# thodson-usgs/discontinuum

Hardware: AMD Instinct MI355X
Metric: GP fits/sec (NLL+grad step) at n=8192 d=3, 1/2/4/8 MI355X (higher is better)
Workload: dtype f64

## Files before the change

discontinuum_amd/_lib.py:

```python
from __future__ import annotations

import ctypes as C
import os

_HERE = os.path.dirname(os.path.abspath(__file__))
LIB_PATH = os.path.join(_HERE, "libdgp_hip.so")

F64, F32 = 0, 1
MODEL_LOADEST, MODEL_RATING = 0, 1
OUT_NLL, OUT_QUAD, OUT_LOGDET, OUT_INFO, OUT_DTHETA, OUT_SUM_DR, OUT_DR_W0, OUT_SUM_DNOISE, OUT_LEN = 0, 1, 2, 3, 4, 28, 29, 31, 32
BUF_XT, BUF_A, BUF_T, BUF_S, BUF_Z, BUF_ALPHA = range(6)
BUF_SCAL = 7
OPT_LAUUM64_MAX_TILES, OPT_SYRK_SLOTS, OPT_TRTRI_SMALL, OPT_REFINE, OPT_SYRK_ORDER, OPT_LAUUM_ORDER, OPT_CHAIN_YIELD, OPT_FUSED_GRAD, OPT_GROUP_GEMM = range(9)
TIME_GRAM, TIME_POTRF, TIME_SYRK_SUM, TIME_SYRK_N, TIME_TRTRI, TIME_LAUUM, TIME_SOLVE, TIME_GRAD, TIME_SYRK_FLOP, TIME_COUNT = range(10)


class DGPLibraryError(RuntimeError):
    pass


class DGPError(RuntimeError):
    def __init__(self, code, where, msg):
        super().__init__(f"{where} failed with code {code}: {msg}")
        self.code = code


_vp, _i, _i64, _sz = C.c_void_p, C.c_int, C.c_int64, C.c_size_t
_dp = C.POINTER(C.c_double)

SIGNATURES = {
    "dgp_version": (_i, []),
    "dgp_last_error": (C.c_char_p, []),
    "dgp_model_ntheta": (_i, [_i, _i]),
    "dgp_composite_define": (_i, [C.POINTER(_i), _i, C.POINTER(_i)]),
    "dgp_padded_n": (_i64, [_i64]),
    "dgp_plan_create": (_i, [_i, _i, _i64, _i, C.POINTER(_vp)]),
    "dgp_plan_destroy": (_i, [_vp]),
    "dgp_plan_workspace_bytes": (_sz, [_vp]),
    "dgp_plan_set_workspace": (_i, [_vp, _vp, _sz]),
    "dgp_plan_set_lookahead": (_i, [_vp, _i]),
    "dgp_plan_set_option": (_i, [_vp, _i, _i64]),
    "dgp_plan_get_option": (_i, [_vp, _i, C.POINTER(_i64)]),
    "dgp_plan_set_batch": (_i, [_vp, _i]),
    "dgp_plan_batch": (_i, [_vp]),
    "dgp_plan_set_site_sizes": (_i, [_vp, C.POINTER(C.c_int64), _vp]),
    "dgp_plan_set_dr_weights": (_i, [_vp, _vp]),
    "dgp_dist_last_error": (C.c_char_p, []),
    "dgp_dist_create": (_i, [_i, _i, _i64, _i, _i, _i, _i, C.POINTER(_vp)]),
    "dgp_dist_destroy": (_i, [_vp]),
    "dgp_dist_padded_n": (_i64, [_vp]),
    "dgp_dist_groups": (_i, [_vp]),
    "dgp_dist_slab_columns": (_i64, [_vp]),
    "dgp_dist_workspace_bytes": (_sz, [_vp]),
    "dgp_dist_panel_elems": (_sz, [_vp, _i]),
    "dgp_dist_set_workspace": (_i, [_vp, _vp, _sz]),
    "dgp_dist_set_inputs": (_i, [_vp, _vp, _vp]),
    "dgp_dist_gram": (_i, [_vp, _dp, _vp, _vp]),
    "dgp_dist_factor": (_i, [_vp, _i, _vp, _vp]),
    "dgp_dist_update": (_i, [_vp, _i, _vp, _i, _i, _vp]),
    "dgp_dist_invert": (_i, [_vp, _i, _vp, _vp]),
    "dgp_dist_status": (_i, [_vp, _vp, _vp]),
    "dgp_dist_solve_partial": (_i, [_vp, _vp, _vp, _vp]),
    "dgp_dist_alpha_partial": (_i, [_vp, _vp, _vp, _vp]),
    "dgp_dist_residual": (_i, [_vp, _dp, _vp, _vp, _vp, _vp, _vp, _vp]),
    "dgp_dist_pack_inverse": (_i, [_vp, _i, _vp, _vp]),
    "dgp_dist_product": (_i, [_vp, _i, _vp, _vp]),
# ... 63 lines not shown
```

discontinuum_amd/csrc/dgp_api.hip:

```cpp
#include <mutex>
#include <new>
#include <stdio.h>
#include <stdlib.h>
#include <string.h>
#include <utility>
#include <vector>

#include "../../include/dgp_hip.h"
#include "dgp_common.h"
#include "dgp_internal.h"

using namespace dgp;

static thread_local char g_err[256] = "";
static int fail(int code, const char* msg) {
  snprintf(g_err, sizeof(g_err), "%s", msg);
  return code;
}
static int hipfail(hipError_t e, const char* where) {
  snprintf(g_err, sizeof(g_err), "%s: %s", where, hipGetErrorString(e));
  return (int)e;
}

struct PinnedRing {
// ... 228 lines not shown
  p->z = p->ws + L.z;
  p->alpha = p->ws + L.alpha;
  p->gpart = p->ws + L.gpart;
  p->spart = p->ws + L.spart;
  p->scal = p->ws + L.scal;
  p->info = (int*)(p->ws + L.info);
  p->snap = p->ws + L.snap;
  p->pre = pre_scratch_bytes(p->B) ? (void*)(p->ws + L.total * (size_t)p->B) : nullptr;
  p->pre2 = p->pre ? (void*)((char*)p->pre + align_up(pre_scratch_bytes(p->B))) : nullptr;
  p->nsite = nullptr;
  p->dr_w = nullptr;
  if (p->B > 1) {
    p->nsite = (int*)(p->ws + L.total * (size_t)p->B + 2 * align_up(pre_scratch_bytes(p->B)));
    delete[] p->nsite_host;
    p->nsite_host = new (std::nothrow) int[(size_t)p->B];
    if (!p->nsite_host) return fail(DGP_E_ARG, "dgp_plan_set_workspace: out of host memory");
    for (int b = 0; b < p->B; ++b) p->nsite_host[b] = (int)p->n;
    hipError_t e = hipMemcpy(p->nsite, p->nsite_host, sizeof(int) * (size_t)p->B, hipMemcpyHostToDevice);
    if (e != hipSuccess) return hipfail(e, "dgp_plan_set_workspace: hipMemcpy");
  }
  p->have_inputs = p->have_factor = 0;
  return 0;
}

int dgp_plan_set_option(dgp_plan* p, int key, int64_t value) {
  if (!p) return fail(DGP_E_ARG, "dgp_plan_set_option: null plan");
  switch (key) {
    case DGP_OPT_LAUUM64_MAX_TILES:
      if (value < 0 || value > (1 << 30)) return fail(DGP_E_ARG, "dgp_plan_set_option: value out of range");
      p->tune.lauum64_max_tiles = (int)value;
      return 0;
    case DGP_OPT_SYRK_SLOTS:
      if (value < 1 || value > (1 << 20)) return fail(DGP_E_ARG, "dgp_plan_set_option: value out of range");
      p->tune.syrk_slots = (int)value;
      return 0;
    case DGP_OPT_TRTRI_SMALL:
      if (value < 0) return fail(DGP_E_ARG, "dgp_plan_set_option: value out of range");
      p->tune.trtri_small = (long)value;
      return 0;
    case DGP_OPT_SYRK_ORDER:
    case DGP_OPT_LAUUM_ORDER:
      if (value < 0 || value > 64) return fail(DGP_E_ARG, "dgp_plan_set_option: value out of range");
      (key == DGP_OPT_SYRK_ORDER ? p->tune.syrk_super : p->tune.lauum_super) = (int)value;
      return 0;
    case DGP_OPT_CHAIN_YIELD:
      p->tune.chain_yield = value ? 1 : 0;
      return 0;
    case DGP_OPT_FUSED_GRAD:
      p->tune.fused_grad = value ? 1 : 0;
      return 0;
    case DGP_OPT_GROUP_GEMM:
      p->tune.group_gemm = value ? 1 : 0;
      return 0;
    case DGP_OPT_REFINE:
      if (p->dtype != DGP_F32 && value) return fail(DGP_E_ARG, "dgp_plan_set_option: refinement applies to float32 plans");
      p->refine = value ? 1 : 0;
      return 0;
    default:
      return fail(DGP_E_ARG, "dgp_plan_set_option: unknown option");
  }
}
int dgp_plan_get_option(const dgp_plan* p, int key, int64_t* value) {
  if (!p || !value) return fail(DGP_E_ARG, "dgp_plan_get_option: null argument");
  switch (key) {
    case DGP_OPT_LAUUM64_MAX_TILES: *value = p->tune.lauum64_max_tiles; return 0;
    case DGP_OPT_SYRK_SLOTS: *value = p->tune.syrk_slots; return 0;
    case DGP_OPT_TRTRI_SMALL: *value = p->tune.trtri_small; return 0;
    case DGP_OPT_REFINE: *value = p->refine; return 0;
    case DGP_OPT_SYRK_ORDER: *value = p->tune.syrk_super; return 0;
    case DGP_OPT_LAUUM_ORDER: *value = p->tune.lauum_super; return 0;
    case DGP_OPT_CHAIN_YIELD: *value = p->tune.chain_yield; return 0;
    case DGP_OPT_FUSED_GRAD: *value = p->tune.fused_grad; return 0;
    case DGP_OPT_GROUP_GEMM: *value = p->tune.group_gemm; return 0;
    default: return fail(DGP_E_ARG, "dgp_plan_get_option: unknown option");
  }
}

int dgp_plan_set_lookahead(dgp_plan* p, int level) {
  if (!p) return fail(DGP_E_ARG, "null plan");
  p->lookahead = level ? default_lookahead() : 0;
  p->early = level >= 2 && !getenv("DGP_NO_EARLY_TRTRI");
  return 0;
}

size_t dgp_plan_site_stride_bytes(const dgp_plan* p) { return p ? layout(p).total : 0; }

int dgp_plan_buffer(const dgp_plan* p, int which, void** dev_ptr, int64_t* ld) {
  if (!p || !dev_ptr || !p->ws) return fail(DGP_E_ARG, "dgp_plan_buffer: null / no workspace");
  void* q = nullptr;
  switch (which) {
    case DGP_BUF_XT: q = p->Xt; break;
    case DGP_BUF_A: q = p->A; break;
    case DGP_BUF_T: q = p->Tm; break;
    case DGP_BUF_S: q = p->S; break;
    case DGP_BUF_Z: q = p->z; break;
    case DGP_BUF_ALPHA: q = p->alpha; break;
    case DGP_BUF_INFO: q = p->info; break;
    case DGP_BUF_SCAL: q = p->scal; break;
    default: return fail(DGP_E_ARG, "dgp_plan_buffer: unknown buffer");
  }
  *dev_ptr = q;
  if (ld) *ld = p->N;
  return 0;
}

}

struct StreamSet {
  hipStream_t bulk = nullptr, rest = nullptr, early = nullptr;
};
static StreamSet* stream_set(hipStream_t caller) {
  static std::mutex mtx;
  static std::vector<std::pair<std::pair<int, hipStream_t>, StreamSet*>> sets;
  int dev = 0;
  if (hipGetDevice(&dev) != hipSuccess) return nullptr;
  std::lock_guard<std::mutex> lock(mtx);
  for (auto& e : sets)
    if (e.first.first == dev && e.first.second == caller) return e.second;
  StreamSet* st = new (std::nothrow) StreamSet();
  if (!st) return nullptr;
  sets.push_back({{dev, caller}, st});
  return st;
}
static int make_stream(hipStream_t* out, bool high) {
  if (*out) return 0;
  int least = 0, greatest = 0;
// ... 844 lines not shown
```

discontinuum_amd/csrc/dgp_chol.hip:

```cpp
#include <stdlib.h>
#include <string.h>
#include <mutex>
#include "dgp_diag.h"
#include "dgp_gemm.h"
#include "dgp_gemm_dma.h"
#include "dgp_internal.h"

namespace dgp {

static constexpr int NB = DGP_TILE;
static constexpr int SMID_TABLE = 4096;
template <typename T>
struct Prefetch {
  static constexpr bool F64 = sizeof(T) == 8;
  static constexpr int LAUUM = F64 ? 2 : 4, TRTRI = F64 ? 1 : 4, SYRK = F64 ? 1 : 2;
};

#define DGP_INFO_CHAIN_TIMEOUT (-7)
#define CHAIN_WAIT_TICKS 200000000LL
__device__ __forceinline__ bool chain_reached(const int* word, int value) {
  return __hip_atomic_load(word, __ATOMIC_RELAXED, __HIP_MEMORY_SCOPE_AGENT) >= value;
}
__device__ __forceinline__ bool chain_wait(const int* w0, int v0, const int* w1, int v1, int* info) {
  __shared__ int chain_ok;
  if (threadIdx.x == 0) {
    int ok = 1;
    if (!(chain_reached(w0, v0) && (w1 == nullptr || chain_reached(w1, v1)))) {
      const long long t0 = wall_clock64();
      while (!(chain_reached(w0, v0) && (w1 == nullptr || chain_reached(w1, v1)))) {
        if (__hip_atomic_load(info + CHAIN_ABORT, __ATOMIC_RELAXED, __HIP_MEMORY_SCOPE_AGENT) != 0) {
          ok = 0;
          break;
        }
        if (wall_clock64() - t0 > CHAIN_WAIT_TICKS) {
          atomicCAS(info, 0, DGP_INFO_CHAIN_TIMEOUT);
          __hip_atomic_store(info + CHAIN_ABORT, 1, __ATOMIC_RELAXED, __HIP_MEMORY_SCOPE_AGENT);
          ok = 0;
          break;
        }
        __builtin_amdgcn_s_sleep(8);
      }
    }
    chain_ok = ok;
  }
  __syncthreads();
  __builtin_amdgcn_fence(__ATOMIC_ACQUIRE, "agent");
  return chain_ok != 0;
}

template <typename T>
__global__ __launch_bounds__(256, 2) void trsm_kernel(T* __restrict__ A, const T* __restrict__ Tinv, long ld, int k,
                                                      long bs, int* __restrict__ wait_info = nullptr, int wait_value = 0) {
  if (wait_info && !chain_wait(wait_info + CHAIN_DIAG_DONE, wait_value, nullptr, 0, wait_info)) return;
  A = site(A, bs);
  Tinv = site(Tinv, bs);
  using G = TileGemm<T, true, true, 64, 128>;
  __shared__ T smem[G::SMEM_ELEMS];
  __builtin_amdgcn_s_setprio(3);
  const long row0 = (long)(k + 1) * NB + (long)blockIdx.x * 64;
// ... 31 lines not shown
  typename G::acc_t keep[G::MI][G::NI];
  constexpr bool STREAM = (CMODE & 1) != 0, WIDE = (CMODE & 2) != 0;
  trailing_begin<T, G, K::DMA, STREAM, WIDE>(acc, keep, C, ld);
  if constexpr (POLITE)
    K::run_hooked(A + row0 * ld + (long)k * NB, ld, A + col0 * ld + (long)k * NB, ld, nk * (NB / 16), smem, acc, YieldHook{yield_word, me, yield_copy});
  else
    K::run(A + row0 * ld + (long)k * NB, ld, A + col0 * ld + (long)k * NB, ld, nk * (NB / 16), smem, acc);
  trailing_end<T, G, K::DMA, STREAM, WIDE>(acc, keep, C, ld);
}

template <typename T, bool POLITE = false, int CMODE = 0, int RING = 3>
__global__ __launch_bounds__(256, (TileCore<T, true, true>::OCC)) void syrk_kernel(T* __restrict__ A, long ld, int k, int nk, int jbeg, int nfull,
                                                                                   int split, long bs, int nt = 0, int super = 0,
                                                                                   const unsigned* yield_word = nullptr) {
  A = site(A, bs);
  __shared__ T smem[TileCore<T, true, true, 128, 128, 1, true, false, RING>::SMEM_ELEMS];
  static_assert(TileCore<T, true, true, 64, 128>::SMEM_ELEMS <= TileCore<T, true, true, 128, 128, 1, true, false, RING>::SMEM_ELEMS &&
                    TileCore<T, true, true, 64, 64>::SMEM_ELEMS <= TileCore<T, true, true, 128, 128, 1, true, false, RING>::SMEM_ELEMS,
                "the cut remainder's register-staged tiles must fit the ring's LDS");
  __shared__ unsigned yield_copy[POLITE ? 4 * 64 : 1];
  const int b = (int)blockIdx.x;
  int bi, bj;
  if (b < nfull) {
    if (super > 0) super_decode(xcd_remap(b, nfull), nt, super, bi, bj);
    else tri_decode(xcd_remap(b, nfull), bi, bj);
    syrk_tile<T, 128, 128, POLITE, CMODE, RING>(A, ld, k, nk, (long)(bi + jbeg) * NB, (long)(bj + jbeg) * NB, smem, yield_word, POLITE ? cu_code() : 0u,
                                   yield_copy + (POLITE ? 64 * __builtin_amdgcn_readfirstlane((int)threadIdx.x >> 6) : 0));
    return;
  }
  const int sub = b - nfull;
  if (super > 0) super_decode(nfull + sub / split, nt, super, bi, bj);
  else tri_decode(nfull + sub / split, bi, bj);
  const long row0 = (long)(bi + jbeg) * NB, col0 = (long)(bj + jbeg) * NB;
  const int part = sub % split;
  if (split == 2) {
    syrk_tile<T, 64, 128, false, CMODE>(A, ld, k, nk, row0 + 64 * part, col0, smem);
  } else {
    if (bi == bj && part == 1) return;
    syrk_tile<T, 64, 64, false, CMODE>(A, ld, k, nk, row0 + 64 * (part >> 1), col0 + 64 * (part & 1), smem);
  }
}

const Tuning& default_tuning() {
  static const Tuning t = [] {
    Tuning v;
    v.lauum64_max_tiles = getenv("DGP_LAUUM64") ? atoi(getenv("DGP_LAUUM64")) : 1000;
    v.syrk_slots = getenv("DGP_SYRK_SLOTS") ? atoi(getenv("DGP_SYRK_SLOTS")) : 512;
    v.trtri_small = getenv("DGP_TRTRI_SMALL") ? atol(getenv("DGP_TRTRI_SMALL")) : 1024;
    v.syrk_super = getenv("DGP_SYRK_ORDER") ? atoi(getenv("DGP_SYRK_ORDER")) : 0;
    v.lauum_super = getenv("DGP_LAUUM_ORDER") ? atoi(getenv("DGP_LAUUM_ORDER")) : 0;
    v.chain_yield = getenv("DGP_CHAIN_YIELD") ? atoi(getenv("DGP_CHAIN_YIELD")) : 1;
    v.fused_grad = getenv("DGP_FUSED_GRAD") ? atoi(getenv("DGP_FUSED_GRAD")) : 0;
    v.group_gemm = getenv("DGP_GROUP_GEMM") ? atoi(getenv("DGP_GROUP_GEMM")) : 0;
    if (v.syrk_slots < 1) v.syrk_slots = 1;
    return v;
  }();
  return t;
}
struct SyrkShape {
  int nfull, split;
  unsigned grid;
  explicit SyrkShape(int ntiles, int slots = 512) {
    if (slots < 1) slots = 1;
    const double cost[5] = {0, 1.0, 0.55, 0, 0.30};
    const int whole = ntiles / slots * slots, rem = ntiles - whole;
    nfull = ntiles;
    split = 1;
    double best = (ntiles + slots - 1) / slots * cost[1];
    for (int g = 2; g <= 4; g += 2) {
      const double c = whole / slots * cost[1] + (g * rem + slots - 1) / slots * cost[g];
      if (rem > 0 && c < best - 1e-9) {
        best = c;
        nfull = whole;
        split = g;
      }
    }
    grid = (unsigned)(nfull + split * (ntiles - nfull));
  }
};

template <typename T>
__global__ __launch_bounds__(256, 2) void syrk_col_kernel(T* __restrict__ A, long ld, int k, int nk, int jcol, int nbk,
                                                          int ncol, long bs) {
  using G = TileGemm<T, true, true, 64, 64>;
  __shared__ T smem[G::SMEM_ELEMS];
  __builtin_amdgcn_s_setprio(3);
  A += (long)((int)blockIdx.z / ncol) * bs;
  const int jc = jcol + (int)blockIdx.z % ncol;
  if ((int)blockIdx.x >= 2 * (nbk - jc)) return;
  const long row0 = (long)jc * NB + (long)blockIdx.x * 64;
  const long col0 = (long)jc * NB + (long)blockIdx.y * 64;
  if (col0 > row0 + 63) return;
  typename G::acc_t acc[G::MI][G::NI];
  T* C = A + row0 * ld + col0;
  typename G::acc_t keep[G::MI][G::NI];
  trailing_begin<T, G>(acc, keep, C, ld);
  G::run(A + row0 * ld + (long)k * NB, ld, A + col0 * ld + (long)k * NB, ld, nk * (NB / 16), smem, acc);
  trailing_end<T, G>(acc, keep, C, ld);
}

template <typename T, int CMODE = 0>
__global__ __launch_bounds__(256, (TileCore<T, true, true>::OCC)) void syrk_col128_kernel(T* __restrict__ A, long ld, int k, int nk, int jcol,
                                                                                          int nbk, int ncol, long bs) {
  __shared__ T smem[TileCore<T, true, true>::SMEM_ELEMS];
  A += (long)((int)blockIdx.z / ncol) * bs;
  const int jc = jcol + (int)blockIdx.z % ncol;
  if ((int)blockIdx.x >= nbk - jc) return;
  syrk_tile<T, 128, 128, false, CMODE>(A, ld, k, nk, (long)(jc + (int)blockIdx.x) * NB, (long)jc * NB, smem);
}

struct DeviceOnce {
  std::mutex mtx;
  bool seen[64] = {false};
  template <typename F>
  hipError_t run(F&& configure) {
    int dev = 0;
    if (hipGetDevice(&dev) != hipSuccess || dev < 0 || dev >= 64) return configure();
    std::lock_guard<std::mutex> lock(mtx);
    if (seen[dev]) return hipSuccess;
    const hipError_t e = configure();
    if (e == hipSuccess) seen[dev] = true;
    return e;
  }
};
static bool f32_diag64() {
  static const bool v = [] {
    const char* e = getenv("DGP_F32_DIAG64");
    return e ? atoi(e) != 0 : false;
  }();
  return v;
}
static bool yields(const Batch& bt) { return bt.B == 1 && bt.tuning().chain_yield != 0; }
template <typename T>
static void launch_bulk(T* A, long N, int k, int nk, int jbeg, const SyrkShape& sh, int nt, int* info, hipStream_t s, const Batch& bt) {
  const int nbk = (int)(N / NB);
  const dim3 grid(sh.grid, 1, (unsigned)bt.B);
  static const int pad_env = getenv("DGP_BULK_LDS_PAD") ? std::min(16384, std::max(0, atoi(getenv("DGP_BULK_LDS_PAD")))) : 14336;
  const size_t pad = (bt.B == 1 && nbk >= 40 && nbk <= 160) ? (size_t)pad_env : 0;
  static const int cmode_env = getenv("DGP_BULK_C") ? atoi(getenv("DGP_BULK_C")) & 3 : DGP_BULK_C_DEFAULT;
  const int cmode = sizeof(T) == 8 ? cmode_env : (cmode_env & 1);
  const unsigned* yw = reinterpret_cast<const unsigned*>(info + CHAIN_YIELD);
  static const int ring_env = getenv("DGP_BULK_RING") ? atoi(getenv("DGP_BULK_RING")) : 3;
  static const int pad_batch = getenv("DGP_BULK_PAD_BATCH") ? std::min(65536, std::max(0, atoi(getenv("DGP_BULK_PAD_BATCH")))) : 0;
  if (bt.B >= 4 && bt.tuning().group_gemm && bt.W != nullptr && ring_env == 2) {
    syrk_kernel<T, false, 0, 2><<<grid, 256, (size_t)pad_batch, s>>>(A, N, k, nk, jbeg, sh.nfull, sh.split, bt.ws, nt, bt.tuning().syrk_super, nullptr);
    return;
  }
  const size_t lds_pad = (bt.B >= 4 && pad_batch > 0) ? (size_t)pad_batch : pad;
#define DGP_LAUNCH_BULK(POLITE_, CM_)                                                                                              \
  syrk_kernel<T, POLITE_, CM_><<<grid, 256, lds_pad, s>>>(A, N, k, nk, jbeg, sh.nfull, sh.split, bt.ws, nt, bt.tuning().syrk_super, \
                                                         POLITE_ ? yw : nullptr)
  if (yields(bt)) {
    switch (cmode) {
      case 1: DGP_LAUNCH_BULK(true, 1); break;
      case 2: DGP_LAUNCH_BULK(true, 2); break;
      case 3: DGP_LAUNCH_BULK(true, 3); break;
      default: DGP_LAUNCH_BULK(true, 0);
    }
  } else {
    switch (cmode) {
      case 1: DGP_LAUNCH_BULK(false, 1); break;
      case 2: DGP_LAUNCH_BULK(false, 2); break;
      case 3: DGP_LAUNCH_BULK(false, 3); break;
      default: DGP_LAUNCH_BULK(false, 0);
    }
  }
#undef DGP_LAUNCH_BULK
}
template <typename TS, typename TC>
static void launch_diag_as(TS* A, long N, long k0, TS* Tinv, TS* logdet, int* info, hipStream_t s, Batch bt, bool init,
                           double* logdet_hi, int done_index, int done_value) {
  const size_t bytes = potrf_diag_fast_smem<TC>();
  static DeviceOnce configured;
  (void)configured.run([&] {
    return hipFuncSetAttribute(reinterpret_cast<const void*>(&potrf_diag_fast_kernel<TS, TC>),
                               hipFuncAttributeMaxDynamicSharedMemorySize, (int)bytes);
  });
  potrf_diag_fast_kernel<TS, TC><<<dim3(1, 1, (unsigned)bt.B), 256, bytes, s>>>(
      A, N, k0, Tinv, logdet, info, bt.ws, bt.ws * (long)sizeof(TS) / (long)sizeof(int), init ? 1 : 0, POTRF_INFO_INTS, logdet_hi,
      done_index, done_value, yields(bt) ? CHAIN_YIELD : -1);
}
template <typename T>
static double* logdet_hi_slot(T* logdet) {
  return sizeof(T) == 4 ? reinterpret_cast<double*>(logdet + 2) : nullptr;
}
template <typename T>
static void launch_diag(T* A, long N, long k0, T* Tinv, T* logdet, int* info, hipStream_t s, Batch bt, bool init = false,
                        int done_index = -1, int done_value = 0) {
  if (sizeof(T) == 4 && f32_diag64())
    launch_diag_as<T, double>(A, N, k0, Tinv, logdet, info, s, bt, init, logdet_hi_slot(logdet), done_index, done_value);
  else
    launch_diag_as<T, T>(A, N, k0, Tinv, logdet, info, s, bt, init, logdet_hi_slot(logdet), done_index, done_value);
}

template <typename T>
__global__ __launch_bounds__(256, (TileCore<T, true, true>::OCC)) void trsm_group_kernel(T* __restrict__ A, const T* __restrict__ Tm, long ld,
                                                                                         int k0, int G, long bs) {
  A = site(A, bs);
  Tm = site(Tm, bs);
  using K = TileCore<T, true, true, 128, 128, 1>;
  using Gm = typename K::G;
  __shared__ T smem[K::SMEM_ELEMS];
  T* Arow = A + (long)(k0 + G + (int)blockIdx.x) * NB * ld + (long)k0 * NB;
  const T* TD = Tm + (long)k0 * NB * ld + (long)k0 * NB;
#pragma unroll 1
  for (int j = G - 1; j >= 0; --j) {
    typename Gm::acc_t acc[Gm::MI][Gm::NI];
    Gm::zero(acc);
    K::run(Arow, ld, TD + (long)j * NB * ld, ld, (j + 1) * (NB / 16), smem, acc);
    T* out = Arow + (long)j * NB;
    K::foreach (acc, [&](int r, int c, T& v) { out[(long)r * ld + c] = v; });
  }
}
template <typename T>
static void trtri_group(const T* L, T* Tm, T* W, long N, int k0, int G, hipStream_t s, Batch bt);

template <typename T>
int potrf(T* A, long N, T* Tinv, T* logdet, int* info, int lookahead, hipStream_t s, hipStream_t s2, hipEvent_t* ev,
          hipEvent_t* syrk_ev, int* n_syrk, double* syrk_flop, int nck, const int* ck_blocks, hipEvent_t* ck_ev,
          void (*on_ck)(void*, int), void* ck_ctx, Batch bt, int q_stop, PotrfCarry* carry) {
  const int nbk = (int)(N / NB);
  int ck_next = carry ? carry->ck_next : 0;
  auto checkpoint = [&](int cols_final) {
    while (ck_next < nck && ck_blocks[ck_next] <= cols_final) {
      hipEventRecord(ck_ev[ck_next], s);
      if (on_ck) on_ck(ck_ctx, ck_next);
      ++ck_next;
    }
  };
  int ns = 0;
  double flop = 0.0;
  const unsigned Bz = (unsigned)bt.B;
  auto tri = [](int m) { return (unsigned)(m * (m + 1) / 2); };
  const double tile_flop = 2.0 * NB * NB * NB;
  if (!lookahead || nbk < 4 || s2 == nullptr || ev == nullptr) {
    for (int k = 0; k < nbk; ++k) {
      launch_diag<T>(A, N, (long)k * NB, Tinv, logdet, info, s, bt, k == 0);
      if (k + 1 < nbk) {
        trsm_kernel<T><<<dim3(2 * (nbk - k - 1), 1, Bz), 256, 0, s>>>(A, Tinv, N, k, bt.ws);
        if (syrk_ev) hipEventRecord(syrk_ev[2 * ns], s);
        {
          const SyrkShape sh((int)tri(nbk - k - 1), bt.tuning().syrk_slots / bt.B);
          syrk_kernel<T><<<dim3(sh.grid, 1, Bz), 256, 0, s>>>(A, N, k, 1, k + 1, sh.nfull, sh.split, bt.ws, nbk - k - 1, bt.tuning().syrk_super);
        }
        if (syrk_ev) hipEventRecord(syrk_ev[2 * ns + 1], s);
        flop += tile_flop * tri(nbk - k - 1) * bt.B;
        ++ns;
      }
    }
    checkpoint(nbk);
    if (n_syrk) *n_syrk = ns;
    if (syrk_flop) *syrk_flop = flop;
    return (int)hipGetLastError();
  }
  {
    const int G = lookahead < 2 ? 2 : (lookahead > 8 ? 8 : lookahead);
    hipEvent_t* P = ev;
    hipEvent_t* U = ev + nbk;
    const int Q = (nbk + G - 1) / G;
    const int Qrun = (q_stop >= 0 && q_stop < Q) ? q_stop : Q;
    for (int q = 0; q < Qrun; ++q) {
      const int k0 = G * q, ncol = nbk - k0 < G ? nbk - k0 : G;
      if (q >= 2) hipStreamWaitEvent(s, U[q - 2], 0);
      if (q >= 1) {
        static const int col128 = getenv("DGP_COL128") ? atoi(getenv("DGP_COL128")) : 4;
        if (bt.B >= col128) {
          static const int ccol = getenv("DGP_COL_C") ? atoi(getenv("DGP_COL_C")) & 3 : DGP_COL_C_DEFAULT;
          const dim3 cgrid(nbk - k0, 1, ncol * Bz);
          switch (sizeof(T) == 8 ? ccol : (ccol & 1)) {
            case 1: syrk_col128_kernel<T, 1><<<cgrid, 256, 0, s>>>(A, N, k0 - G, G, k0, nbk, ncol, bt.ws); break;
            case 2: syrk_col128_kernel<T, 2><<<cgrid, 256, 0, s>>>(A, N, k0 - G, G, k0, nbk, ncol, bt.ws); break;
            case 3: syrk_col128_kernel<T, 3><<<cgrid, 256, 0, s>>>(A, N, k0 - G, G, k0, nbk, ncol, bt.ws); break;
            default: syrk_col128_kernel<T, 0><<<cgrid, 256, 0, s>>>(A, N, k0 - G, G, k0, nbk, ncol, bt.ws);
          }
        }
        else syrk_col_kernel<T><<<dim3(2 * (nbk - k0), 2, ncol * Bz), 256, 0, s>>>(A, N, k0 - G, G, k0, nbk, ncol, bt.ws);
      }
      if (q >= 1 && k0 + G < nbk) {
        hipEventRecord(P[q - 1], s);
        hipStreamWaitEvent(s2, P[q - 1], 0);
        if (syrk_ev) hipEventRecord(syrk_ev[2 * ns], s2);
        {
          const SyrkShape sh((int)tri(nbk - k0 - G), bt.tuning().syrk_slots / bt.B);
          launch_bulk<T>(A, N, k0 - G, G, k0 + G, sh, nbk - k0 - G, info, s2, bt);
        }
        if (syrk_ev) hipEventRecord(syrk_ev[2 * ns + 1], s2);
        flop += (double)G * tile_flop * tri(nbk - k0 - G) * bt.B;
        ++ns;
        hipEventRecord(U[q - 1], s2);
      }
      const bool group_gemm = bt.tuning().group_gemm && bt.W != nullptr && ncol == G && k0 + G < nbk && (G & (G - 1)) == 0 && G >= 4 &&
                              nck == 0;
      const int kend = group_gemm ? k0 + G : nbk;
      for (int h = 0; h < ncol; ++h) {
        const int k = k0 + h;
        if (h >= 1) syrk_col_kernel<T><<<dim3(2 * (kend - k), 2, Bz), 256, 0, s>>>(A, N, k0, h, k, kend, 1, bt.ws);
        launch_diag<T>(A, N, (long)k * NB, Tinv, logdet, info, s, bt, k == 0);
        if (k + 1 < kend) trsm_kernel<T><<<dim3(2 * (kend - k - 1), 1, Bz), 256, 0, s>>>(A, Tinv, N, k, bt.ws);
        if (!group_gemm) checkpoint(k + 1);
      }
      if (group_gemm) {
        trtri_group<T>(A, Tinv, (T*)bt.W, N, k0, G, s, bt);
        trsm_group_kernel<T><<<dim3((unsigned)(nbk - k0 - G), 1, Bz), 256, 0, s>>>(A, Tinv, N, k0, G, bt.ws);
        checkpoint(k0 + G);
      }
    }
    if (Qrun == Q) checkpoint(nbk);
// ... 923 lines not shown
```

discontinuum_amd/csrc/dgp_internal.h:

```cpp
#pragma once
#include <hip/hip_runtime.h>
#include <stdint.h>

#define DGP_TILE_HOST 128

namespace dgp {

inline long round_up(long n, long q) { return (n + q - 1) / q * q; }

#define DGP_MAX_BATCH_HOST 8
#define DGP_MAX_BATCH_SITES 1024
struct Tuning {
  int lauum64_max_tiles;
  int syrk_slots;
  long trtri_small;
  int syrk_super;
  int lauum_super;
  int chain_yield;
  int fused_grad;
  int group_gemm;
};
const Tuning& default_tuning();
struct Batch {
  int B = 1;
  long ws = 0;
  const int* ns = nullptr;
  const Tuning* tune = nullptr;
  void* W = nullptr;
  const Tuning& tuning() const { return tune ? *tune : default_tuning(); }
};
int model_ntheta(int model, int d);
int composite_define(const int* spec, int nspec);
bool composite_select(int model, int d);

template <typename T>
int pack_x(const T* X, int n, int d, long N, T* Xt, hipStream_t s, Batch bt = Batch());
template <typename T>
int gram_sym(int model, int d, const T* Xt, long N, int n, const double* theta, const T* noise, T* K, hipStream_t s,
             Batch bt = Batch(), void* pre_scratch = nullptr ,
             void* pre_staging = nullptr ,
             long k_stride = -1 , long noise_stride = -1 ,
             bool pre_ready = false );
template <typename T>
int gram_cross(int model, int d, const T* Xt, long N, int n, const T* Xst, long M, int m, const double* theta,
               T* Ks, hipStream_t s, Batch bt = Batch(), long wbs = 0, void* pre_scratch = nullptr, void* pre_staging = nullptr);
template <typename T>
int gram_diag(int model, int d, const T* Xst, long M, int m, const double* theta, T* kss, hipStream_t s, Batch bt = Batch(),
              long wbs = 0, void* pre_scratch = nullptr);
template <typename T>
int gram_grad(int model, int d, const T* Xt, long N, int n, const double* theta, const T* S, const T* alpha,
              T* partials, T* dtheta, hipStream_t s, Batch bt = Batch(), long dtheta_stride = 0,
              void* pre_scratch = nullptr, bool pre_ready = false ,
              void* pre_staging = nullptr);
size_t pre_scratch_bytes(int B);
template <typename TS>
int gram_residual(int model, int d, const TS* Xt, long N, int n, const double* theta, const TS* noise, const TS* r,
                  const TS* alpha, double* part, double* rho64, TS* rho32, hipStream_t s, Batch bt, long ps, long rs,
                  void* pre_scratch, void* pre_staging);
size_t gram_residual_scratch_bytes(long N);
long gram_grad_partials(long N);
bool lauum_grad_applies(int model, long N, const Batch& bt);
template <typename T>
int lauum_grad(int model, int d, const T* Tm, long N, T* S, const T* Xt, int n, const double* theta, const T* alpha, T* partials,
               T* dtheta, hipStream_t s, Batch bt, long dtheta_stride, void* pre_scratch, bool pre_ready, void* pre_staging);
template <typename T>
int mean_vjp_grad(int model, int d, const T* Xt, long N, int n, const T* Xst, long Mp, int m, const double* theta,
                  const T* alpha, const T* beta, const T* wts, T* partials, T* dtheta, hipStream_t s, Batch bt = Batch(),
                  long wbs = 0, long dstride = 0, void* pre_scratch = nullptr, void* pre_staging = nullptr);
template <typename T>
int gemv_rows(const T* Ks, long N, long Mp, int m, const T* w, T* out, hipStream_t s, int B = 1, long wbs = 0);

struct PotrfCarry {
  int ck_next = 0, ns = 0;
  double flop = 0.0;
};
// ... 87 lines not shown
```

include/dgp_hip.h:

```cpp
#ifndef DGP_HIP_H
#define DGP_HIP_H
#include <stddef.h>
#include <stdint.h>

#ifdef __cplusplus
extern "C" {
#endif

#define DGP_F64 0
#define DGP_F32 1
#define DGP_MODEL_LOADEST 0
#define DGP_MODEL_RATING 1

#define DGP_E_ARG (-1)
#define DGP_E_MODEL (-2)
#define DGP_E_WORKSPACE (-3)
#define DGP_E_STATE (-4)

#define DGP_OUT_NLL 0
#define DGP_OUT_QUAD 1
#define DGP_OUT_LOGDET 2
#define DGP_OUT_INFO 3
#define DGP_OUT_DTHETA 4
#define DGP_OUT_SUM_DR 28
#define DGP_OUT_DR_W0 29
#define DGP_OUT_SUM_DNOISE 31
#define DGP_OUT_LEN 32

#define DGP_BUF_XT 0
#define DGP_BUF_A 1
#define DGP_BUF_T 2
#define DGP_BUF_S 3
#define DGP_BUF_Z 4
#define DGP_BUF_ALPHA 5
#define DGP_BUF_INFO 6
#define DGP_BUF_SCAL 7

typedef struct dgp_plan dgp_plan;

int dgp_version(void);
const char* dgp_last_error(void);
int dgp_model_ntheta(int model, int d);
int dgp_composite_define(const int* spec_host, int nspec, int* model_out);
int64_t dgp_padded_n(int64_t n);

int dgp_plan_create(int model, int dtype, int64_t n, int d, dgp_plan** out);
int dgp_plan_destroy(dgp_plan* plan);
size_t dgp_plan_workspace_bytes(const dgp_plan* plan);
int dgp_plan_set_batch(dgp_plan* plan, int batch);
int dgp_plan_batch(const dgp_plan* plan);
int dgp_plan_set_site_sizes(dgp_plan* plan, const int64_t* sizes_host, void* stream);
int dgp_plan_set_workspace(dgp_plan* plan, void* dev_ptr, size_t bytes);
int dgp_plan_set_dr_weights(dgp_plan* plan, const void* w_dev);
int dgp_plan_set_lookahead(dgp_plan* plan, int level);
#define DGP_OPT_LAUUM64_MAX_TILES 0
#define DGP_OPT_SYRK_SLOTS 1
#define DGP_OPT_TRTRI_SMALL 2
#define DGP_OPT_REFINE 3
#define DGP_OPT_SYRK_ORDER 4
#define DGP_OPT_LAUUM_ORDER 5
#define DGP_OPT_CHAIN_YIELD 6
#define DGP_OPT_FUSED_GRAD 7
#define DGP_OPT_GROUP_GEMM 8
int dgp_plan_set_option(dgp_plan* plan, int key, int64_t value);
int dgp_plan_get_option(const dgp_plan* plan, int key, int64_t* value_out);
int dgp_plan_buffer(const dgp_plan* plan, int which, void** dev_ptr, int64_t* ld);
size_t dgp_plan_site_stride_bytes(const dgp_plan* plan);

int dgp_set_inputs(dgp_plan* plan, const void* X_dev, void* stream);

int dgp_fit_step(dgp_plan* plan, const double* theta_host, const void* r_dev, const void* noise_dev,
                 void* out_dev, void* dr_dev, void* dnoise_dev, void* stream);

int dgp_factorize(dgp_plan* plan, const double* theta_host, const void* r_dev, const void* noise_dev,
                  void* out_dev, void* stream);

size_t dgp_predict_workspace_bytes(const dgp_plan* plan, int64_t m);
int dgp_predict(dgp_plan* plan, const double* theta_host, const void* Xs_dev, int64_t m, void* work_dev,
                size_t work_bytes, void* mean_dev, void* var_dev, void* stream);

int dgp_posterior_cov(dgp_plan* plan, const double* theta_host, const void* Xs_dev, int64_t m, void* work_dev,
                      size_t work_bytes, void* mean_dev, void* cov_dev, void* stream);

int dgp_sample_draws(int dtype, const void* L_dev, int64_t m, const void* Z_dev, int64_t ndraw, const void* mean_dev,
                     void* out_dev, void* stream);

size_t dgp_period_moments_workspace_bytes(int64_t m, int ngroups, int batch);
int dgp_period_moments(int dtype, int mode, const void* cov_dev, int64_t m, int batch, const void* mu_dev,
                       const double* scale2_dev, const double* w_dev, const int32_t* group_dev, int ngroups,
                       const void* extra_var_dev, void* work_dev, size_t work_bytes, double* mean_out_dev,
                       double* cov_out_dev, void* stream);

size_t dgp_posterior_period_moments_workspace_bytes(const dgp_plan* plan, int64_t m, int ngroups);
int dgp_posterior_period_moments(dgp_plan* plan, const double* theta_host, const void* Xs_dev, int64_t m, int mode,
                                 const void* mu_dev, const double* scale2_dev, const double* w_dev,
                                 const int32_t* group_dev, int ngroups, const void* extra_var_dev,
                                 void* work_dev, size_t work_bytes, double* mean_out_dev, double* cov_out_dev,
                                 void* stream);

size_t dgp_cross_validate_workspace_bytes(const dgp_plan* plan, int ngroups, int64_t max_group);
int dgp_cross_validate(dgp_plan* plan, const int32_t* order_dev, const int32_t* start_dev, int ngroups, int64_t max_group,
                       void* work_dev, size_t work_bytes, double* resid_dev, double* var_dev, double* lpd_dev, int32_t* info_dev,
                       void* stream);

size_t dgp_mean_vjp_workspace_bytes(const dgp_plan* plan, int64_t m);
int dgp_predict_mean(dgp_plan* plan, const double* theta_host, const void* Xs_dev, int64_t m, void* work_dev,
                     size_t work_bytes, void* mean_dev, void* stream);
int dgp_mean_vjp(dgp_plan* plan, const double* theta_host, const void* Xs_dev, int64_t m, const void* w_dev,
                 void* work_dev, size_t work_bytes, void* dtheta_dev, void* dr_dev, void* dnoise_dev, void* stream);

#define DGP_TIME_GRAM 0
#define DGP_TIME_POTRF 1
#define DGP_TIME_SYRK_SUM 2
#define DGP_TIME_SYRK_N 3
#define DGP_TIME_TRTRI 4
#define DGP_TIME_LAUUM 5
// ... 53 lines not shown
```

Baseline: 109.4.

## Add a schedule-driven left-looking blocked Cholesky path for large f64 batches

Adds a small scheduler that emits a left-looking op list (strip SYRK updates, panel factorisations, optional grouped triangular solves, and syncs across two streams), plus a validator that checks the dependencies. A new strip SYRK kernel runs each update as one launch over the triangle and rectangle tiles of a column strip. The path turns on automatically for f64 plans with batch of at least 32 and more than 4 block columns, replacing the existing right-looking lookahead loop. The aim is fewer, larger update launches and better overlap between the two streams. In exchange it adds host-side op generation and a dependency check on every call, and the new path is only reached for large batches.

```diff
diff --git a/discontinuum_amd/_lib.py b/discontinuum_amd/_lib.py
--- a/discontinuum_amd/_lib.py
+++ b/discontinuum_amd/_lib.py
@@ -12,6 +12,7 @@
 BUF_XT, BUF_A, BUF_T, BUF_S, BUF_Z, BUF_ALPHA = range(6)
 BUF_SCAL = 7
 OPT_LAUUM64_MAX_TILES, OPT_SYRK_SLOTS, OPT_TRTRI_SMALL, OPT_REFINE, OPT_SYRK_ORDER, OPT_LAUUM_ORDER, OPT_CHAIN_YIELD, OPT_FUSED_GRAD, OPT_GROUP_GEMM = range(9)
+OPT_POTRF_SCHEDULE, OPT_POTRF_SWEEP, OPT_POTRF_SOLVE, OPT_POTRF_OVERLAP, OPT_POTRF_SLOTS, OPT_POTRF_TAIL, OPT_POTRF_TAIL_SWEEP = range(9, 16)
 TIME_GRAM, TIME_POTRF, TIME_SYRK_SUM, TIME_SYRK_N, TIME_TRTRI, TIME_LAUUM, TIME_SOLVE, TIME_GRAD, TIME_SYRK_FLOP, TIME_COUNT = range(10)
 
 
diff --git a/discontinuum_amd/csrc/dgp_api.hip b/discontinuum_amd/csrc/dgp_api.hip
--- a/discontinuum_amd/csrc/dgp_api.hip
+++ b/discontinuum_amd/csrc/dgp_api.hip
@@ -304,6 +304,26 @@
     case DGP_OPT_GROUP_GEMM:
       p->tune.group_gemm = value ? 1 : 0;
       return 0;
+    case DGP_OPT_POTRF_SCHEDULE:
+      if (value < 0 || value > 1) return fail(DGP_E_ARG, "dgp_plan_set_option: value out of range");
+      p->tune.potrf_schedule = (int)value;
+      return 0;
+    case DGP_OPT_POTRF_SWEEP:
+    case DGP_OPT_POTRF_TAIL:
+    case DGP_OPT_POTRF_TAIL_SWEEP:
+      if (value < 0 || value > (1 << 20)) return fail(DGP_E_ARG, "dgp_plan_set_option: value out of range");
+      (key == DGP_OPT_POTRF_SWEEP ? p->tune.potrf_sweep : key == DGP_OPT_POTRF_TAIL ? p->tune.potrf_tail : p->tune.potrf_tail_sweep) = (int)value;
+      return 0;
+    case DGP_OPT_POTRF_SOLVE:
+      p->tune.potrf_solve = value ? 1 : 0;
+      return 0;
+    case DGP_OPT_POTRF_OVERLAP:
+      p->tune.potrf_overlap = value ? 1 : 0;
+      return 0;
+    case DGP_OPT_POTRF_SLOTS:
+      if (value < 1 || value > (1 << 20)) return fail(DGP_E_ARG, "dgp_plan_set_option: value out of range");
+      p->tune.potrf_slots = (int)value;
+      return 0;
     case DGP_OPT_REFINE:
       if (p->dtype != DGP_F32 && value) return fail(DGP_E_ARG, "dgp_plan_set_option: refinement applies to float32 plans");
       p->refine = value ? 1 : 0;
@@ -324,6 +344,15 @@
     case DGP_OPT_CHAIN_YIELD: *value = p->tune.chain_yield; return 0;
     case DGP_OPT_FUSED_GRAD: *value = p->tune.fused_grad; return 0;
     case DGP_OPT_GROUP_GEMM: *value = p->tune.group_gemm; return 0;
+    case DGP_OPT_POTRF_SCHEDULE:
+      *value = p->tune.potrf_schedule < 0 ? (p->B >= 4 ? potrf_schedule_auto(p->B, p->N / DGP_TILE_HOST, p->elem) : 0) : p->tune.potrf_schedule;
+      return 0;
+    case DGP_OPT_POTRF_SWEEP: *value = p->tune.potrf_sweep; return 0;
+    case DGP_OPT_POTRF_SOLVE: *value = p->tune.potrf_solve; return 0;
+    case DGP_OPT_POTRF_OVERLAP: *value = p->tune.potrf_overlap; return 0;
+    case DGP_OPT_POTRF_SLOTS: *value = p->tune.potrf_slots; return 0;
+    case DGP_OPT_POTRF_TAIL: *value = p->tune.potrf_tail; return 0;
+    case DGP_OPT_POTRF_TAIL_SWEEP: *value = p->tune.potrf_tail_sweep; return 0;
     default: return fail(DGP_E_ARG, "dgp_plan_get_option: unknown option");
   }
 }
diff --git a/discontinuum_amd/csrc/dgp_chol.hip b/discontinuum_amd/csrc/dgp_chol.hip
--- a/discontinuum_amd/csrc/dgp_chol.hip
+++ b/discontinuum_amd/csrc/dgp_chol.hip
@@ -1,10 +1,12 @@
 #include <stdlib.h>
 #include <string.h>
+#include <algorithm>
 #include <mutex>
 #include "dgp_diag.h"
 #include "dgp_gemm.h"
 #include "dgp_gemm_dma.h"
 #include "dgp_internal.h"
+#include "dgp_schedule.h"
 
 namespace dgp {
 
@@ -142,11 +144,19 @@
     v.chain_yield = getenv("DGP_CHAIN_YIELD") ? atoi(getenv("DGP_CHAIN_YIELD")) : 1;
     v.fused_grad = getenv("DGP_FUSED_GRAD") ? atoi(getenv("DGP_FUSED_GRAD")) : 0;
     v.group_gemm = getenv("DGP_GROUP_GEMM") ? atoi(getenv("DGP_GROUP_GEMM")) : 0;
+    v.potrf_schedule = getenv("DGP_POTRF_SCHEDULE") ? (atoi(getenv("DGP_POTRF_SCHEDULE")) != 0 ? 1 : 0) : -1;
+    v.potrf_sweep = getenv("DGP_POTRF_SWEEP") ? std::max(0, atoi(getenv("DGP_POTRF_SWEEP"))) : 0;
+    v.potrf_tail = getenv("DGP_POTRF_TAIL") ? std::max(0, atoi(getenv("DGP_POTRF_TAIL"))) : 0;
+    v.potrf_tail_sweep = getenv("DGP_POTRF_TAIL_SWEEP") ? std::max(0, atoi(getenv("DGP_POTRF_TAIL_SWEEP"))) : 0;
+    v.potrf_solve = getenv("DGP_POTRF_SOLVE") ? atoi(getenv("DGP_POTRF_SOLVE")) : 0;
+    v.potrf_overlap = getenv("DGP_POTRF_OVERLAP") ? atoi(getenv("DGP_POTRF_OVERLAP")) : 0;
+    v.potrf_slots = getenv("DGP_POTRF_SLOTS") ? std::max(1, atoi(getenv("DGP_POTRF_SLOTS"))) : 768;
     if (v.syrk_slots < 1) v.syrk_slots = 1;
     return v;
   }();
   return t;
 }
+int potrf_schedule_auto(int B, long nbk, int elem) { return (elem == 8 && B >= 32 && nbk > 4) ? 1 : 0; }
 struct SyrkShape {
   int nfull, split;
   unsigned grid;
@@ -199,6 +209,39 @@
   syrk_tile<T, 128, 128, false, CMODE>(A, ld, k, nk, (long)(jc + (int)blockIdx.x) * NB, (long)jc * NB, smem);
 }
 
+template <typename T>
+__global__ __launch_bounds__(256, (TileCore<T, true, true>::OCC)) void syrk_strip_kernel(T* __restrict__ A, long ld, int k, int nk, int c0, int ncol,
+                                                                                         int rrect, int ntri, int nt, int nfull, int split, long bs) {
+  __shared__ T smem[TileCore<T, true, true>::SMEM_ELEMS];
+  static_assert(TileCore<T, true, true, 64, 128>::SMEM_ELEMS <= TileCore<T, true, true>::SMEM_ELEMS &&
+                    TileCore<T, true, true, 64, 64>::SMEM_ELEMS <= TileCore<T, true, true>::SMEM_ELEMS,
+                "the cut remainder's register-staged tiles must fit the ring's LDS");
+  const int b = (int)blockIdx.x;
+  const int l = b < nfull ? xcd_remap(b, nfull) : nfull + (b - nfull) / split;
+  const int t = l % nt;
+  A += (long)(l / nt) * bs;
+  int bi, bj;
+  if (t < ntri) {
+    tri_decode(t, bi, bj);
+    bi += c0;
+  } else {
+    bi = rrect + (t - ntri) / ncol;
+    bj = (t - ntri) % ncol;
+  }
+  const long row0 = (long)bi * NB, col0 = (long)(c0 + bj) * NB;
+  if (b < nfull) {
+    syrk_tile<T, 128, 128>(A, ld, k, nk, row0, col0, smem);
+    return;
+  }
+  const int part = (b - nfull) % split;
+  if (split == 2) {
+    syrk_tile<T, 64, 128>(A, ld, k, nk, row0 + 64 * part, col0, smem);
+  } else {
+    if (row0 == col0 && part == 1) return;
+    syrk_tile<T, 64, 64>(A, ld, k, nk, row0 + 64 * (part >> 1), col0 + 64 * (part & 1), smem);
+  }
+}
+
 struct DeviceOnce {
   std::mutex mtx;
   bool seen[64] = {false};
@@ -304,6 +347,70 @@
 }
 template <typename T>
 static void trtri_group(const T* L, T* Tm, T* W, long N, int k0, int G, hipStream_t s, Batch bt);
+
+template <typename T>
+static int potrf_scheduled(T* A, long N, T* Tinv, T* logdet, int* info, int G, hipStream_t s, hipStream_t s2, hipEvent_t* ev,
+                           hipEvent_t* syrk_ev, int* n_syrk, double* syrk_flop, const Batch& bt) {
+  const int nbk = (int)(N / NB);
+  sched::Cut cut;
+  cut.sweep = bt.tuning().potrf_sweep;
+  cut.tail = bt.tuning().potrf_tail;
+  cut.tail_sweep = bt.tuning().potrf_tail_sweep;
+  cut.solve = bt.tuning().potrf_solve && bt.W != nullptr;
+  cut.overlap = bt.tuning().potrf_overlap;
+  const std::vector<sched::Op> ops = sched::left_looking(nbk, G, cut);
+  if (!sched::check(ops, nbk).empty()) return (int)hipErrorInvalidValue;
+  const unsigned Bz = (unsigned)bt.B;
+  const double tile_flop = 2.0 * NB * NB * NB;
+  hipStream_t st[2] = {s, s2};
+  int ns = 0, nsync = 0;
+  double flop = 0.0;
+  for (const sched::Op& o : ops) {
+    hipStream_t so = st[o.stream];
+    switch (o.kind) {
+      case sched::SYNC:
+        hipEventRecord(ev[nsync], so);
+        hipStreamWaitEvent(st[o.c0], ev[nsync], 0);
+        ++nsync;
+        break;
+      case sched::UPDATE: {
+        const long nt = sched::update_tiles(o);
+        const bool timed = syrk_ev != nullptr && ns < nbk;
+        if (timed) hipEventRecord(syrk_ev[2 * ns], so);
+        {
+          const SyrkShape sh((int)(nt * bt.B), bt.tuning().potrf_slots);
+          const int ncol = o.c1 - o.c0, h = (o.r0 == o.c0) ? std::min(o.r1, o.c1) - o.c0 : 0;
+          syrk_strip_kernel<T><<<dim3(sh.grid, 1, 1), 256, 0, so>>>(A, N, o.ka, o.kb - o.ka, o.c0, ncol, std::max(o.r0, o.c1), h * (h + 1) / 2, (int)nt,
+                                                                     sh.nfull, sh.split, bt.ws);
+        }
+        if (timed) {
+          hipEventRecord(syrk_ev[2 * ns + 1], so);
+          flop += tile_flop * (double)nt * (o.kb - o.ka) * bt.B;
+          ++ns;
+        }
+        break;
+      }
+      case sched::PANELS:
+        for (int k = o.c0; k < o.c1; ++k) {
+          if (k > o.c0) syrk_col_kernel<T><<<dim3(2 * (o.r1 - k), 2, Bz), 256, 0, so>>>(A, N, o.c0, k - o.c0, k, o.r1, 1, bt.ws);
+          launch_diag<T>(A, N, (long)k * NB, Tinv, logdet, info, so, bt, k == 0);
+          if (k + 1 < o.r1) trsm_kernel<T><<<dim3(2 * (o.r1 - k - 1), 1, Bz), 256, 0, so>>>(A, Tinv, N, k, bt.ws);
+        }
+        break;
+      case sched::SOLVE:
+        trtri_group<T>(A, Tinv, (T*)bt.W, N, o.c0, o.c1 - o.c0, so, bt);
+        trsm_group_kernel<T><<<dim3((unsigned)(o.r1 - o.r0), 1, Bz), 256, 0, so>>>(A, Tinv, N, o.c0, o.c1 - o.c0, bt.ws);
+        break;
+    }
+  }
+  if (n_syrk) *n_syrk = ns;
+  if (syrk_flop) *syrk_flop = flop;
+  return (int)hipGetLastError();
+}
+static bool scheduled_applies(const Batch& bt, long nbk, int elem, int G, int nck, int q_stop, const PotrfCarry* carry, hipStream_t s2, hipEvent_t* ev) {
+  const int mode = bt.tuning().potrf_schedule < 0 ? potrf_schedule_auto(bt.B, nbk, elem) : bt.tuning().potrf_schedule;
+  return bt.B >= 4 && mode != 0 && G >= 4 && nbk > G && nck == 0 && q_stop < 0 && carry == nullptr && s2 != nullptr && ev != nullptr;
+}
 
 template <typename T>
 int potrf(T* A, long N, T* Tinv, T* logdet, int* info, int lookahead, hipStream_t s, hipStream_t s2, hipEvent_t* ev,
@@ -343,6 +450,8 @@
     if (syrk_flop) *syrk_flop = flop;
     return (int)hipGetLastError();
   }
+  if (scheduled_applies(bt, nbk, (int)sizeof(T), lookahead, nck, q_stop, carry, s2, ev))
+    return potrf_scheduled<T>(A, N, Tinv, logdet, info, lookahead > 8 ? 8 : lookahead, s, s2, ev, syrk_ev, n_syrk, syrk_flop, bt);
   {
     const int G = lookahead < 2 ? 2 : (lookahead > 8 ? 8 : lookahead);
     hipEvent_t* P = ev;
diff --git a/discontinuum_amd/csrc/dgp_internal.h b/discontinuum_amd/csrc/dgp_internal.h
--- a/discontinuum_amd/csrc/dgp_internal.h
+++ b/discontinuum_amd/csrc/dgp_internal.h
@@ -19,8 +19,16 @@
   int chain_yield;
   int fused_grad;
   int group_gemm;
+  int potrf_schedule;
+  int potrf_sweep;
+  int potrf_tail;
+  int potrf_tail_sweep;
+  int potrf_solve;
+  int potrf_slots;
+  int potrf_overlap;
 };
 const Tuning& default_tuning();
+int potrf_schedule_auto(int B, long nbk, int elem);
 struct Batch {
   int B = 1;
   long ws = 0;
diff --git a/discontinuum_amd/csrc/dgp_schedule.h b/discontinuum_amd/csrc/dgp_schedule.h
--- /dev/null
+++ b/discontinuum_amd/csrc/dgp_schedule.h
@@ -0,0 +1,182 @@
+#pragma once
+#include <string>
+#include <vector>
+
+namespace dgp {
+namespace sched {
+
+enum Kind { UPDATE = 0, PANELS = 1, SOLVE = 2, SYNC = 3 };
+struct Op {
+  int kind, stream;
+  int c0, c1;
+  int r0, r1;
+  int ka, kb;
+};
+struct Cut {
+  int sweep = 0;
+  int tail = 0;
+  int tail_sweep = 0;
+  int solve = 0;
+  int overlap = 0;
+};
+inline bool sweep_point(int nbk, int G, int c, const Cut& cut) {
+  if (c <= 0 || c >= nbk) return false;
+  const int S = cut.sweep > 0 ? (cut.sweep + G - 1) / G * G : 0, St = cut.tail_sweep > 0 ? (cut.tail_sweep + G - 1) / G * G : 0;
+  const int t0 = cut.tail > 0 ? (nbk - cut.tail) / G * G : 0;
+  if (t0 > 0 && c >= t0) return c == t0 || (St > 0 && (c - t0) % St == 0);
+  return S > 0 && c % S == 0;
+}
+
+inline bool solves(int nbk, int G, int k0, const Cut& cut) {
+  const int c1 = k0 + G < nbk ? k0 + G : nbk;
+  return cut.solve && c1 - k0 == G && c1 < nbk && G >= 4 && (G & (G - 1)) == 0;
+}
+
+inline std::vector<Op> today(int nbk, int G) {
+  std::vector<Op> ops;
+  const int Q = (nbk + G - 1) / G;
+  for (int q = 0; q < Q; ++q) {
+    const int k0 = G * q, c1 = k0 + G < nbk ? k0 + G : nbk;
+    if (q >= 2) ops.push_back({SYNC, 1, 0, 0, 0, 0, 0, 0});
+    if (q >= 1) ops.push_back({UPDATE, 0, k0, c1, k0, nbk, k0 - G, k0});
+    if (q >= 1 && k0 + G < nbk) {
+      ops.push_back({SYNC, 0, 1, 0, 0, 0, 0, 0});
+      ops.push_back({UPDATE, 1, k0 + G, nbk, k0 + G, nbk, k0 - G, k0});
+    }
+    ops.push_back({PANELS, 0, k0, c1, k0, nbk, 0, 0});
+  }
+  return ops;
+}
+
+inline std::vector<Op> left_looking(int nbk, int G, const Cut& cut) {
+  std::vector<Op> ops;
+  bool forked = false;
+  int base = 0;
+  for (int k0 = 0; k0 < nbk; k0 += G) {
+    const int c1 = k0 + G < nbk ? k0 + G : nbk;
+    const bool solve = solves(nbk, G, k0, cut);
+    bool split = false;
+    if (k0 > base) {
+      if (solve && cut.overlap) {
+        split = true;
+        ops.push_back({UPDATE, 0, k0, c1, k0, c1, base, k0});
+        ops.push_back({SYNC, 0, 1, 0, 0, 0, 0, 0});
+        ops.push_back({UPDATE, 1, k0, c1, c1, nbk, base, k0});
+        forked = true;
+      } else {
+        ops.push_back({UPDATE, 0, k0, c1, k0, nbk, base, k0});
+      }
+    }
+    ops.push_back({PANELS, 0, k0, c1, k0, solve ? c1 : nbk, 0, 0});
+    if (solve) {
+      if (split) {
+        ops.push_back({SYNC, 1, 0, 0, 0, 0, 0, 0});
+        forked = false;
+      }
+      ops.push_back({SOLVE, 0, k0, c1, c1, nbk, 0, 0});
+    }
+    if (sweep_point(nbk, G, c1, cut)) {
+      ops.push_back({UPDATE, 0, c1, nbk, c1, nbk, base, c1});
+      base = c1;
+    }
+  }
+  if (forked) ops.push_back({SYNC, 1, 0, 0, 0, 0, 0, 0});
+  return ops;
+}
+
+inline long update_tiles(const Op& o) {
+  long t = 0;
+  for (int j = o.c0; j < o.c1; ++j) {
+    const int lo = o.r0 > j ? o.r0 : j;
+    if (o.r1 > lo) t += o.r1 - lo;
+  }
+  return t;
+}
+
+inline std::string check(const std::vector<Op>& ops, int nbk) {
+  auto at = [nbk](int i, int j) { return (size_t)i * nbk + j; };
+  std::vector<int> applied((size_t)nbk * nbk, 0), wstream((size_t)nbk * nbk, -1), wclock((size_t)nbk * nbk, 0);
+  std::vector<char> fin((size_t)nbk * nbk, 0);
+  int clock[2] = {0, 0}, seen[2][2] = {{0, 0}, {0, 0}};
+  auto where = [](size_t n, const Op& o) {
+    return "op " + std::to_string(n) + " (kind " + std::to_string(o.kind) + ", columns " + std::to_string(o.c0) + ".." + std::to_string(o.c1) +
+           ", rows " + std::to_string(o.r0) + ".." + std::to_string(o.r1) + ", k " + std::to_string(o.ka) + ".." + std::to_string(o.kb) + "): ";
+  };
+  for (size_t n = 0; n < ops.size(); ++n) {
+    const Op& o = ops[n];
+    if (o.stream < 0 || o.stream > 1) return where(n, o) + "bad stream";
+    const int X = o.stream;
+    auto visible = [&](int i, int j) { return wstream[at(i, j)] < 0 || wstream[at(i, j)] == X || seen[X][wstream[at(i, j)]] >= wclock[at(i, j)]; };
+    auto readable = [&](int i, int k) { return fin[at(i, k)] && visible(i, k); };
+    if (o.kind == SYNC) {
+      if (o.c0 < 0 || o.c0 > 1 || o.c0 == X) return where(n, o) + "bad SYNC";
+      seen[o.c0][X] = clock[X];
+      continue;
+    }
+    if (o.c0 < 0 || o.c1 > nbk || o.c0 >= o.c1 || o.r0 < o.c0 || o.r1 > nbk) return where(n, o) + "out of range";
+    const int now = ++clock[X];
+    auto write = [&](int i, int j) {
+      wstream[at(i, j)] = X;
+      wclock[at(i, j)] = now;
+    };
+    if (o.kind == UPDATE) {
+      if (o.ka < 0 || o.ka >= o.kb || o.kb > o.c0) return where(n, o) + "k-range must lie left of the columns";
+      if (update_tiles(o) == 0) return where(n, o) + "empty";
+      for (int j = o.c0; j < o.c1; ++j)
+        for (int i = (o.r0 > j ? o.r0 : j); i < o.r1; ++i) {
+          if (fin[at(i, j)]) return where(n, o) + "writes a final block";
+          if (applied[at(i, j)] != o.ka)
+            return where(n, o) + "tile (" + std::to_string(i) + ", " + std::to_string(j) + ") has received " + std::to_string(applied[at(i, j)]) + " k-blocks";
+          if (!visible(i, j)) return where(n, o) + "tile written on the other stream without a SYNC";
+          for (int k = o.ka; k < o.kb; ++k)
+            if (!readable(i, k) || !readable(j, k)) return where(n, o) + "reads block column " + std::to_string(k) + " before it is final";
+          applied[at(i, j)] = o.kb;
+        }
+      for (int j = o.c0; j < o.c1; ++j)
+        for (int i = (o.r0 > j ? o.r0 : j); i < o.r1; ++i) write(i, j);
+    } else if (o.kind == PANELS) {
+      if (o.r0 != o.c0 || o.r1 < o.c1) return where(n, o) + "PANELS covers its diagonal block";
+      for (int j = o.c0; j < o.c1; ++j)
+        for (int i = j; i < o.r1; ++i) {
+          if (fin[at(i, j)]) return where(n, o) + "factored twice";
+          if (applied[at(i, j)] != o.c0)
+            return where(n, o) + "tile (" + std::to_string(i) + ", " + std::to_string(j) + ") has received " + std::to_string(applied[at(i, j)]) + " of " + std::to_string(o.c0) + " k-blocks";
+          if (!visible(i, j)) return where(n, o) + "tile written on the other stream without a SYNC";
+        }
+      for (int j = o.c0; j < o.c1; ++j)
+        for (int i = j; i < o.r1; ++i) {
+          applied[at(i, j)] = j;
+          fin[at(i, j)] = 1;
+          write(i, j);
+        }
+    } else if (o.kind == SOLVE) {
+      if (o.r0 != o.c1 || o.r1 != nbk || o.r0 >= o.r1) return where(n, o) + "SOLVE covers the rows below the group's diagonal block";
+      for (int j = o.c0; j < o.c1; ++j)
+        for (int i = j; i < o.c1; ++i)
+          if (!readable(i, j)) return where(n, o) + "the diagonal block is not final";
+      for (int j = o.c0; j < o.c1; ++j)
+        for (int i = o.r0; i < o.r1; ++i) {
+          if (fin[at(i, j)]) return where(n, o) + "solved twice";
+          if (applied[at(i, j)] != o.c0)
+            return where(n, o) + "tile (" + std::to_string(i) + ", " + std::to_string(j) + ") has received " + std::to_string(applied[at(i, j)]) + " of " + std::to_string(o.c0) + " k-blocks";
+          if (!visible(i, j)) return where(n, o) + "tile written on the other stream without a SYNC";
+        }
+      for (int j = o.c0; j < o.c1; ++j)
+        for (int i = o.r0; i < o.r1; ++i) {
+          applied[at(i, j)] = j;
+          fin[at(i, j)] = 1;
+          write(i, j);
+        }
+    } else {
+      return where(n, o) + "unknown kind";
+    }
+  }
+  for (int j = 0; j < nbk; ++j)
+    for (int i = j; i < nbk; ++i)
+      if (!fin[at(i, j)]) return "block (" + std::to_string(i) + ", " + std::to_string(j) + ") is never factored";
+  if (seen[0][1] < clock[1]) return "stream 0 has not joined stream 1 at the end";
+  return "";
+}
+
+}
+}
diff --git a/include/dgp_hip.h b/include/dgp_hip.h
--- a/include/dgp_hip.h
+++ b/include/dgp_hip.h
@@ -62,6 +62,13 @@
 #define DGP_OPT_CHAIN_YIELD 6
 #define DGP_OPT_FUSED_GRAD 7
 #define DGP_OPT_GROUP_GEMM 8
+#define DGP_OPT_POTRF_SCHEDULE 9
+#define DGP_OPT_POTRF_SWEEP 10
+#define DGP_OPT_POTRF_SOLVE 11
+#define DGP_OPT_POTRF_OVERLAP 12
+#define DGP_OPT_POTRF_SLOTS 13
+#define DGP_OPT_POTRF_TAIL 14
+#define DGP_OPT_POTRF_TAIL_SWEEP 15
 int dgp_plan_set_option(dgp_plan* plan, int key, int64_t value);
 int dgp_plan_get_option(const dgp_plan* plan, int key, int64_t* value_out);
 int dgp_plan_buffer(const dgp_plan* plan, int which, void** dev_ptr, int64_t* ld);
```

New measurement: 111.2 (median of 6 runs). 1.02x the previous value.
